# JiehongLin/SAM-6D

Hardware: AMD Instinct MI355X
Metric: RGB-D frames/sec (SAM-6D per-frame hot path: SAM ViT-H encoder + ISM scoring + PEM) (higher is better)
Workload: dtype bf16 (SAM ViT-H: 87 % of the step) + f16 (PEM ViT-B feature extractor) + f32 (ISM scoring, PEM point transformer and pose solvers); 1 GPU; LM-O single object: 32 frames/step/GPU, 640x480 RGB-D -> 1024^2 SAM input, P=128 proposals x 42 templates (scored in groups of 8 frames), 1 instance/frame, 2048 pts (PEM batch 32); sam_frames_per_launch_group=16, pem_vit_dtype=fp16 (set by bench.py; the library default is fp32)

## Files before the change

### sam6d_amd/csrc/s6d_attn_common.h

```cpp
#pragma once
#include "s6d_bf16.h"

#ifndef S6D_ATTN_F16
#define S6D_ATTN_F16 0
#endif
#if S6D_ATTN_F16
#define S6D_ATTN_NS s6d_h
#define S6D_ATTN_MFMA16(a, b, c) __builtin_amdgcn_mfma_f32_16x16x32_f16(a, b, c, 0, 0, 0)
#define S6D_ATTN_ONE 0x3C00
#else
#define S6D_ATTN_NS s6d
#define S6D_ATTN_MFMA16(a, b, c) __builtin_amdgcn_mfma_f32_16x16x32_bf16(a, b, c, 0, 0, 0)
#define S6D_ATTN_ONE 0x3F80
#endif

namespace S6D_ATTN_NS {
using namespace s6d;

#if S6D_ATTN_F16
typedef f16x8 bf16x8;
__device__ __forceinline__ u16 f2bf(float f) {
  union { _Float16 b; u16 u; } x;
  x.b = (_Float16)f;
  return x.u;
}
__device__ __forceinline__ float bf2f(u16 h) {
  union { _Float16 b; u16 u; } x;
  x.u = h;
  return (float)x.b;
}
#else
__device__ __forceinline__ u16 f2bf(float f) { return bf16_bits(f); }
__device__ __forceinline__ float bf2f(u16 h) { return bf16_value(h); }
#endif

struct AttnParams {
  const u16 *qkv;
  const u16 *qkv_bias;
  const u16 *rel_h;
  const u16 *rel_w;
  u16 *out;
  int B, H, W, nh;
  int ws;
  int S;
  int T;
  int nwx, nwy;
  int LT;
  unsigned magicS;
  float scale_log2;
  long tok_stride, which_stride, head_stride;
};

__device__ __forceinline__ const u16 *qkv_at(const AttnParams &p, size_t tok, int which, int head) {
  return p.qkv + tok * (size_t)p.tok_stride + (size_t)which * (size_t)p.which_stride + (size_t)head * (size_t)p.head_stride;
}

#ifndef S6D_ATTN_ABLATE
#define S6D_ATTN_ABLATE 0
#endif
constexpr int kAbl = S6D_ATTN_ABLATE;
#ifndef S6D_G64_TIMING
#define S6D_G64_TIMING 0
#endif
#if S6D_G64_TIMING
#define S6D_TICK(tk, i)                                  \
  do {                                                   \
    __builtin_amdgcn_sched_barrier(0);                   \
    (tk)[i] = (long long)__builtin_amdgcn_s_memtime();   \
    __builtin_amdgcn_sched_barrier(0);                   \
  } while (0)
#else
#define S6D_TICK(tk, i) do { } while (0)
#endif

constexpr float kLog2e = 1.4426950408889634f;
__device__ __forceinline__ float fast_exp2(float x) { return __builtin_amdgcn_exp2f(x); }

template <int HD>
struct Cfg {
  static constexpr int KS = (HD + 31) / 32;
  static constexpr int HDP = KS * 32;
  static constexpr int DT = HD / 16;
  static constexpr int KROW = HDP + 8;
  static constexpr int VROW = HD == 64 ? HD + 8 : (((HD + 15) / 16) | 1) * 16;
  static constexpr int KT = 64;
  static constexpr int KPARTS = HDP / 8, VPARTS = HD / 8;
};

__device__ __forceinline__ int div_S(const AttnParams &p, int n) { return (int)__umulhi((unsigned)n, p.magicS); }

__device__ __forceinline__ bool token_offset(const AttnParams &p, int b, int wy, int wx, int t, size_t &off) {
  if (p.ws == 0) {
    off = (size_t)b * p.T + min(t, p.T - 1);
    return t < p.T;
  }
  const int ty = div_S(p, t), tx = t - ty * p.S;
  const int y = wy * p.ws + ty, x = wx * p.ws + tx;
  const bool in = (y < p.H) && (x < p.W) && (t < p.T);
  off = (in || p.qkv_bias) ? ((size_t)(b * p.H + min(y, p.H - 1)) * p.W + min(x, p.W - 1)) : (size_t)b * p.H * p.W;
  return in;
}

template <int HD>
__device__ __forceinline__ uint4 load_chunk(const AttnParams &p, int which, int head, bool valid, size_t tok, int d0) {
  const int C = p.nh * HD;
  const int dc = d0 < HD ? d0 : HD - 8;
  const u16 *a = qkv_at(p, tok, which, head) + dc;
  const u16 *bsrc = p.qkv_bias ? p.qkv_bias + (size_t)which * C + head * HD + dc : a;
  const uint4 v = *reinterpret_cast<const uint4 *>(valid ? a : bsrc);
  return d0 < HD ? v : make_uint4(0, 0, 0, 0);
}

template <int HD, int NS>
struct StripState {
  bf16x8 qf[NS][Cfg<HD>::KS];
  float twr[NS][16];
  float m_run[NS];
  f32x4 lacc[NS];
  f32x4 oacc[NS][Cfg<HD>::DT];
  const float *th[NS], *tw[NS];
  int qy[NS], qx[NS];
};

template <int HD, int MODE, int NS, bool KSWZ = false, bool PRIO = false, int SUBS = 4>
__device__ __forceinline__ void process_tile(const AttnParams &p, const u16 *Kl, const u16 *Vl, int key0,
                                             StripState<HD, NS> &st, const float (&thv)[NS], int lane, long long *tk = nullptr) {
  using C = Cfg<HD>;
  static_assert(SUBS >= 1 && SUBS <= 4, "a tile has four 16-key sub-tiles");
  const int g = lane >> 4, c = lane & 15;
  const int gk = KSWZ ? (g ^ kswz(c)) : g;
  float s[NS][4][4];
  if (PRIO) __builtin_amdgcn_s_setprio(1);
  auto kfrag = [&](int sub, int ks) __attribute__((always_inline)) {
    return *reinterpret_cast<const bf16x8 *>(Kl + (sub * 16 + c) * C::KROW + ks * 32 + gk * 8);
  };
#pragma unroll
  for (int sub = 0; sub < 4; ++sub) {
    f32x4 acc[NS];
#pragma unroll
    for (int n = 0; n < NS; ++n) acc[n] = f32x4{0.f, 0.f, 0.f, 0.f};
    if (sub >= SUBS) {
#pragma unroll
      for (int n = 0; n < NS; ++n)
#pragma unroll
        for (int r = 0; r < 4; ++r) s[n][sub][r] = -1e30f;
      continue;
    }
    if (!(kAbl & 16)) {
#pragma unroll
      for (int ks = 0; ks < C::KS; ++ks) {
        const bf16x8 a = kfrag(sub, ks);
#pragma unroll
        for (int n = 0; n < NS; ++n) acc[n] = S6D_ATTN_MFMA16(a, st.qf[n][ks], acc[n]);
      }
    }
#pragma unroll
    for (int n = 0; n < NS; ++n)
#pragma unroll
      for (int r = 0; r < 4; ++r) {
        float v = acc[n][r] * p.scale_log2;
        if (MODE == 1) {
          s[n][sub][r] = v + st.twr[n][sub * 4 + r];
        } else {
          const int kk = key0 + sub * 16 + g * 4 + r;
          if (MODE == 0) {
            const int ky = div_S(p, kk), kx = kk - ky * p.S;
            const int jh = min(max(st.qy[n] - ky + p.S - 1, 0), p.LT - 1), jw = st.qx[n] - kx + p.S - 1;
            v += st.th[n][c * p.LT + jh] + st.tw[n][c * p.LT + jw];
          }
          s[n][sub][r] = kk < p.T ? v : -1e30f;
        }
      }
  }
  union PB { bf16x8 v; u16 h[8]; };
  PB pb[NS][2];
  union VA { bf16x8 v; s16x4 q[2]; };
  if (PRIO) __builtin_amdgcn_s_setprio(0);
  if (kAbl & 4) {
#pragma unroll
    for (int n = 0; n < NS; ++n)
#pragma unroll
      for (int sub = 0; sub < 4; ++sub)
#pragma unroll
        for (int r = 0; r < 4; ++r) pb[n][sub >> 1].h[(sub & 1) * 4 + r] = f2bf(s[n][sub][r]);
  } else {
    constexpr float kDefer = 6.0f;
    float mx[NS];
    bool grow[NS], any_grow = false;
#pragma unroll
    for (int n = 0; n < NS; ++n) {
      float v = s[n][0][0];
#pragma unroll
      for (int sub = 0; sub < SUBS; ++sub)
#pragma unroll
        for (int r = 0; r < 4; ++r) v = fmaxf(v, s[n][sub][r]);
      v = fmaxf(v, __shfl_xor(v, 16));
      v = fmaxf(v, __shfl_xor(v, 32));
      if (MODE == 1) v += thv[n];
      mx[n] = v;
      grow[n] = __any(v - st.m_run[n] > kDefer);
      any_grow |= grow[n];
    }
    S6D_TICK(tk, 3);
    if (any_grow) {
#pragma unroll
      for (int n = 0; n < NS; ++n)
        if (grow[n]) {
          const float m_new = fmaxf(st.m_run[n], mx[n]);
          const float alpha = fast_exp2(st.m_run[n] - m_new);
          st.lacc[n] *= alpha;
#pragma unroll
          for (int dt = 0; dt < C::DT; ++dt) st.oacc[n][dt] *= alpha;
          st.m_run[n] = m_new;
        }
    }
#pragma unroll
    for (int n = 0; n < NS; ++n) {
      const float m_sub = (MODE == 1) ? st.m_run[n] - thv[n] : st.m_run[n];
#pragma unroll
      for (int sub = 0; sub < 4; ++sub)
#pragma unroll
        for (int r = 0; r < 4; ++r)
          pb[n][sub >> 1].h[(sub & 1) * 4 + r] = sub < SUBS ? f2bf(fast_exp2(s[n][sub][r] - m_sub)) : (u16)0;
    }
  }
  if (kAbl & 8) {
#pragma unroll
    for (int n = 0; n < NS; ++n) st.lacc[n][0] += (float)pb[n][0].h[0] + (float)pb[n][1].h[7];
    return;
  }
  union { bf16x8 v; u16 h[8]; } ones;
#pragma unroll
  for (int i = 0; i < 8; ++i) ones.h[i] = S6D_ATTN_ONE;
  S6D_TICK(tk, 4);
  if (PRIO) __builtin_amdgcn_s_setprio(1);
#pragma unroll
  for (int j = 0; j < (SUBS + 1) / 2; ++j) {
    const u16 *vrow = Vl + (32 * j + g * 4 + (c >> 2)) * C::VROW + (c & 3) * 4;
#pragma unroll
    for (int n = 0; n < NS; ++n) st.lacc[n] = S6D_ATTN_MFMA16(ones.v, pb[n][j].v, st.lacc[n]);
#pragma unroll
    for (int dt = 0; dt < C::DT; ++dt) {
      VA va;
      va.q[0] = __builtin_amdgcn_ds_read_tr16_b64_v4i16((S6D_LDS(s16x4) *)(vrow + dt * 16));
      va.q[1] = __builtin_amdgcn_ds_read_tr16_b64_v4i16((S6D_LDS(s16x4) *)(vrow + 16 * C::VROW + dt * 16));
#pragma unroll
      for (int n = 0; n < NS; ++n)
        st.oacc[n][dt] = S6D_ATTN_MFMA16(va.v, pb[n][j].v, st.oacc[n][dt]);
    }
  }
  if (PRIO) __builtin_amdgcn_s_setprio(0);
}

constexpr float kNoMaxSumLimit = 1.2676506e30f;
constexpr float kNoMaxFinite = 3.0e38f;

template <int HD, int NS, bool KSWZ>
__device__ __forceinline__ void process_tile_nomax(const AttnParams &p, const u16 *Kl, const u16 *Vl, StripState<HD, NS> &st,
                                                   const f32x4 (&cbias)[NS][4], const float (&nb)[NS], int lane) {
  using C = Cfg<HD>;
  const int g = lane >> 4, c = lane & 15;
  const int gk = KSWZ ? (g ^ kswz(c)) : g;
  union PB { bf16x8 v; u16 h[8]; };
  PB pb[NS][2];
#pragma unroll
  for (int sub = 0; sub < 4; ++sub) {
    f32x4 acc[NS];
#pragma unroll
    for (int n = 0; n < NS; ++n) acc[n] = cbias[n][sub];
#pragma unroll
    for (int ks = 0; ks < C::KS; ++ks) {
      const bf16x8 a = *reinterpret_cast<const bf16x8 *>(Kl + (sub * 16 + c) * C::KROW + ks * 32 + gk * 8);
#pragma unroll
      for (int n = 0; n < NS; ++n) acc[n] = S6D_ATTN_MFMA16(a, st.qf[n][ks], acc[n]);
    }
#pragma unroll
    for (int n = 0; n < NS; ++n)
#pragma unroll
      for (int r = 0; r < 4; ++r)
        pb[n][sub >> 1].h[(sub & 1) * 4 + r] = f2bf(fast_exp2(__builtin_fmaf(acc[n][r], p.scale_log2, nb[n])));
  }
  union { bf16x8 v; u16 h[8]; } ones;
#pragma unroll
  for (int i = 0; i < 8; ++i) ones.h[i] = S6D_ATTN_ONE;
  union VA { bf16x8 v; s16x4 q[2]; };
#pragma unroll
  for (int j = 0; j < 2; ++j) {
    const u16 *vrow = Vl + (32 * j + g * 4 + (c >> 2)) * C::VROW + (c & 3) * 4;
#pragma unroll
    for (int n = 0; n < NS; ++n) st.lacc[n] = S6D_ATTN_MFMA16(ones.v, pb[n][j].v, st.lacc[n]);
#pragma unroll
    for (int dt = 0; dt < C::DT; ++dt) {
      VA va;
      va.q[0] = __builtin_amdgcn_ds_read_tr16_b64_v4i16((S6D_LDS(s16x4) *)(vrow + dt * 16));
      va.q[1] = __builtin_amdgcn_ds_read_tr16_b64_v4i16((S6D_LDS(s16x4) *)(vrow + 16 * C::VROW + dt * 16));
#pragma unroll
      for (int n = 0; n < NS; ++n) st.oacc[n][dt] = S6D_ATTN_MFMA16(va.v, pb[n][j].v, st.oacc[n][dt]);
    }
  }
}

template <int HD, int THREADS>
struct Stager {
  using C = Cfg<HD>;
  static constexpr int NK = (64 * C::KPARTS + THREADS - 1) / THREADS;
  static constexpr int NV = (64 * C::VPARTS + THREADS - 1) / THREADS;
  uint4 k[NK], v[NV];

  __device__ __forceinline__ void load(const AttnParams &p, int b, int wy, int wx, int head, int key0, int tid) {
#pragma unroll
    for (int n = 0; n < NK; ++n) {
      const int i = min(tid + n * THREADS, 64 * C::KPARTS - 1);
      const int key = i / C::KPARTS, part = i - key * C::KPARTS;
      size_t tok;
      const bool valid = token_offset(p, b, wy, wx, key0 + key, tok);
      k[n] = load_chunk<HD>(p, 1, head, valid, tok, part * 8);
    }
#pragma unroll
    for (int n = 0; n < NV; ++n) {
      const int i = min(tid + n * THREADS, 64 * C::VPARTS - 1);
      const int key = i / C::VPARTS, part = i - key * C::VPARTS;
      size_t tok;
      const bool valid = token_offset(p, b, wy, wx, key0 + key, tok);
      v[n] = load_chunk<HD>(p, 2, head, valid, tok, part * 8);
    }
  }
  __device__ __forceinline__ void store(u16 *Kl, u16 *Vl, int tid, int klim = 64, int vlim = 64) const {
#pragma unroll
    for (int n = 0; n < NK; ++n) {
      const int i = tid + n * THREADS;
      const int key = i / C::KPARTS, part = i - key * C::KPARTS;
      if (i < 64 * C::KPARTS && key < klim) *reinterpret_cast<uint4 *>(Kl + key * C::KROW + part * 8) = k[n];
    }
#pragma unroll
    for (int n = 0; n < NV; ++n) {
      const int i = tid + n * THREADS;
      const int key = i / C::VPARTS, part = i - key * C::VPARTS;
      if (i < 64 * C::VPARTS && key < vlim) *reinterpret_cast<uint4 *>(Vl + key * C::VROW + part * 8) = v[n];
    }
  }
};

template <int HD, int THREADS>
struct StagerLinear {
  using C = Cfg<HD>;
  static constexpr int NK = (64 * C::KPARTS + THREADS - 1) / THREADS;
  static constexpr int NV = (64 * C::VPARTS + THREADS - 1) / THREADS;
  uint4 k[NK], v[NV];
  const u16 *kp[NK], *vp[NV];
  int ko[NK], vo[NV];
  bool kz[NK];
  static_assert(Cfg<HD>::KROW - Cfg<HD>::HDP == 8, "K rows end in a 16-byte pad");

  __device__ __forceinline__ void init(const AttnParams &p, int b, int head, int tid) {
#pragma unroll
    for (int n = 0; n < NK; ++n) {
      const int i = tid + n * THREADS, ic = min(i, 64 * C::KPARTS - 1);
      const int key = ic / C::KPARTS, part = ic - key * C::KPARTS;
      kz[n] = part * 8 >= HD;
      kp[n] = qkv_at(p, (size_t)b * p.T + key, 1, head) + (kz[n] ? HD - 8 : part * 8);
      ko[n] = i < 64 * C::KPARTS ? key * C::KROW + (part ^ kswz(key)) * 8 : (tid & 63) * C::KROW + C::HDP;
    }
#pragma unroll
    for (int n = 0; n < NV; ++n) {
      const int i = tid + n * THREADS, ic = min(i, 64 * C::VPARTS - 1);
      const int key = ic / C::VPARTS, part = ic - key * C::VPARTS;
      vp[n] = qkv_at(p, (size_t)b * p.T + key, 2, head) + part * 8;
      vo[n] = i < 64 * C::VPARTS ? 64 * C::KROW + key * C::VROW + part * 8 : (tid & 63) * C::KROW + C::HDP;
    }
  }
  __device__ __forceinline__ void load(size_t tile_stride_elems, int t) {
#pragma unroll
    for (int n = 0; n < NK; ++n) k[n] = *reinterpret_cast<const uint4 *>(kp[n] + tile_stride_elems * t);
#pragma unroll
    for (int n = 0; n < NV; ++n) v[n] = *reinterpret_cast<const uint4 *>(vp[n] + tile_stride_elems * t);
  }
  __device__ __forceinline__ void store(u16 *Kl) const {
#pragma unroll
    for (int n = 0; n < NK; ++n) *reinterpret_cast<uint4 *>(Kl + ko[n]) = kz[n] ? make_uint4(0, 0, 0, 0) : k[n];
#pragma unroll
    for (int n = 0; n < NV; ++n) *reinterpret_cast<uint4 *>(Kl + vo[n]) = v[n];
  }
};

template <int HD>
__device__ __forceinline__ void load_q(const AttnParams &p, int b, int wy, int wx, int head, int q0,
                                       bf16x8 (&qf)[Cfg<HD>::KS], int lane) {
  const int g = lane >> 4, c = lane & 15;
  size_t tok;
  const bool valid = token_offset(p, b, wy, wx, q0 + c, tok);
#pragma unroll
  for (int ks = 0; ks < Cfg<HD>::KS; ++ks) {
    union { uint4 u; bf16x8 v; } x;
    x.u = load_chunk<HD>(p, 0, head, valid, tok, ks * 32 + g * 8);
    qf[ks] = x.v;
  }
}

template <int HD, int NJT>
__device__ __forceinline__ void build_table(const u16 *rel, int j0, int sgn, const bf16x8 (&qf)[Cfg<HD>::KS],
                                            float *dst, int ld, int lane) {
  using C = Cfg<HD>;
  const int g = lane >> 4, c = lane & 15;
  union { uint4 u; bf16x8 v; } r[NJT][C::KS];
#pragma unroll
  for (int jt = 0; jt < NJT; ++jt) {
    const int j = j0 + sgn * (jt * 16 + c);
#pragma unroll
    for (int ks = 0; ks < C::KS; ++ks)
      r[jt][ks].u = *reinterpret_cast<const uint4 *>(rel + (size_t)j * C::HDP + ks * 32 + g * 8);
  }
#pragma unroll
  for (int jt = 0; jt < NJT; ++jt) {
    f32x4 a = {0.f, 0.f, 0.f, 0.f};
#pragma unroll
    for (int ks = 0; ks < C::KS; ++ks) a = S6D_ATTN_MFMA16(r[jt][ks].v, qf[ks], a);
    float *o = dst + c * ld + jt * 16 + g * 4;
    if ((ld & 3) == 0) {
      *reinterpret_cast<float4 *>(o) = make_float4(a[0] * kLog2e, a[1] * kLog2e, a[2] * kLog2e, a[3] * kLog2e);
    } else {
#pragma unroll
      for (int r = 0; r < 4; ++r) o[r] = a[r] * kLog2e;
    }
  }
}

template <int HD>
__device__ __forceinline__ void store_strip(const AttnParams &p, int b, int wy, int wx, int head, int q0, float l_run,
                                            const f32x4 (&oacc)[Cfg<HD>::DT], int lane) {
  const int g = lane >> 4, c = lane & 15;
  size_t tok;
  if (!token_offset(p, b, wy, wx, q0 + c, tok)) return;
  const float inv = 1.0f / l_run;
  u16 *dst = p.out + tok * (size_t)(p.nh * HD) + head * HD;
#pragma unroll
  for (int dt = 0; dt < Cfg<HD>::DT; ++dt) {
    union { uint2 u; u16 h[4]; } o;
#pragma unroll
    for (int r = 0; r < 4; ++r) o.h[r] = f2bf(oacc[dt][r] * inv);
    *reinterpret_cast<uint2 *>(dst + dt * 16 + g * 4) = o.u;
  }
}

struct WinItem {
  int b, wy, wx, head;
  __device__ __forceinline__ void decode(const AttnParams &p, int id) {
    const int nwin = p.B * p.nwy * p.nwx, cut = (nwin & ~7) * p.nh;
    int win;
    if (id < cut) {
      const int xcd = id & 7, loc = id >> 3;
      head = loc % p.nh;
      win = (loc / p.nh) * 8 + xcd;
    } else {
      head = id % p.nh;
      win = id / p.nh;
    }
    wx = win % p.nwx; win /= p.nwx;
    wy = win % p.nwy; win /= p.nwy;
    b = win;
  }
};

__device__ const uint4 g_attn_zero16 = {0u, 0u, 0u, 0u};

template <class... P, class... A>
static void launch_lds(void (*kernel)(P...), unsigned grid, unsigned block, size_t lds, hipStream_t st, A... args) {
  (void)hipFuncSetAttribute(reinterpret_cast<const void *>(kernel), hipFuncAttributeMaxDynamicSharedMemorySize, (int)lds);
  hipLaunchKernelGGL(kernel, dim3(grid), dim3(block), lds, st, args...);
}

}
```

### sam6d_amd/csrc/s6d_attn_global.h

```cpp
#pragma once
#include "s6d_attn_common.h"

namespace S6D_ATTN_NS {

constexpr bool kGlbPrio = true;

template <int HD, int WAVES, int MODE>
__global__ __launch_bounds__(WAVES * 64) void attn_global_kernel(AttnParams p) {
  using C = Cfg<HD>;
  constexpr int NS = 2;
  static_assert(MODE == 0 || MODE == 2, "attn_global_kernel: table bias (0) or no bias (2); the 64 x 64 grid is attn_global64_kernel's");
  S6D_DYN_LDS(smem);
  constexpr int KBYTES = 64 * C::KROW * 2, VBYTES = 64 * C::VROW * 2;
  auto Kbuf = [&](int r) { return reinterpret_cast<u16 *>(smem + r * (KBYTES + VBYTES)); };
  auto Vbuf = [&](int r) { return reinterpret_cast<u16 *>(smem + r * (KBYTES + VBYTES) + KBYTES); };
  float *tabs = reinterpret_cast<float *>(smem + 2 * (KBYTES + VBYTES));
  const int tid = threadIdx.x, wave = tid >> 6, lane = tid & 63;
  const int c = lane & 15;

  const int nqt = (p.T + WAVES * 16 * NS - 1) / (WAVES * 16 * NS);
  int id = blockIdx.x;
  const int nbh = p.B * p.nh;
  int qt, bh;
  if ((nbh & 7) == 0) {
    const int xcd = id & 7, loc = id >> 3;
    qt = loc % nqt;
    bh = (loc / nqt) * 8 + xcd;
  } else {
    qt = id % nqt;
    bh = id / nqt;
  }
  const int head = bh % p.nh, b = bh / p.nh;
  StripState<HD, NS> st;
  int q0[NS];
#pragma unroll
  for (int n = 0; n < NS; ++n) {
    q0[n] = ((qt * WAVES + wave) * NS + n) * 16;
    load_q<HD>(p, b, 0, 0, head, q0[n], st.qf[n], lane);
    const int qi = min(q0[n] + c, p.T - 1);
    st.qy[n] = div_S(p, qi);
    st.qx[n] = qi - st.qy[n] * p.S;
    st.m_run[n] = -1e30f;
    st.lacc[n] = f32x4{0.f, 0.f, 0.f, 0.f};
#pragma unroll
    for (int i = 0; i < 16; ++i) st.twr[n][i] = 0.f;
#pragma unroll
    for (int dt = 0; dt < C::DT; ++dt) st.oacc[n][dt] = f32x4{0.f, 0.f, 0.f, 0.f};
    st.th[n] = nullptr;
    st.tw[n] = nullptr;
  }
  if (MODE == 0) {
#pragma unroll
    for (int n = 0; n < NS; ++n) {
      float *th = tabs + (size_t)(wave * NS + n) * 2 * 16 * p.LT, *tw = th + 16 * p.LT;
      for (int jt = 0; jt < p.LT / 16; ++jt) {
        build_table<HD, 1>(p.rel_h, jt * 16, 1, st.qf[n], th + jt * 16, p.LT, lane);
        build_table<HD, 1>(p.rel_w, jt * 16, 1, st.qf[n], tw + jt * 16, p.LT, lane);
      }
      st.th[n] = th;
      st.tw[n] = tw;
    }
  }
  const int ntile = p.T / 64;
  StagerLinear<HD, WAVES * 64> sg;
  sg.init(p, b, head, tid);
  const size_t tstride = (size_t)64 * (size_t)p.tok_stride;
  sg.load(tstride, 0);
  __syncthreads();
  sg.store(Kbuf(0));
  __syncthreads();
  auto tile = [&](int t) {
    const float thv[NS] = {0.f, 0.f};
    if (!(kAbl & 2)) process_tile<HD, MODE, NS, true, kGlbPrio>(p, Kbuf(t & 1), Vbuf(t & 1), t * 64, st, thv, lane);
  };
  for (int t = 0; t + 1 < ntile; ++t) {
    if (!(kAbl & 1)) sg.load(tstride, t + 1);
    tile(t);
    if (!(kAbl & 32)) sg.store(Kbuf((t & 1) ^ 1));
    __syncthreads();
  }
  tile(ntile - 1);
#pragma unroll
  for (int n = 0; n < NS; ++n) store_strip<HD>(p, b, 0, 0, head, q0[n], st.lacc[n][0], st.oacc[n], lane);
}

constexpr int G64_THLD = 65;
#ifndef S6D_G64_SLOTS
#define S6D_G64_SLOTS 3
#endif
#ifndef S6D_G64_WAVES
#define S6D_G64_WAVES 8
#endif
#ifndef S6D_G64_NOMAX
#define S6D_G64_NOMAX 1
#endif

template <int HD, int WAVES_, int SLOTS_>
struct G64 {
  using C = Cfg<HD>;
  static constexpr int WAVES = WAVES_, NS = 2, SLOTS = SLOTS_;
  static constexpr int KCH = C::KROW / 8, VCH = C::VROW / 8;
  static constexpr int NPIECE = KCH + VCH;
  static constexpr int PW = (NPIECE + WAVES - 1) / WAVES;
  static constexpr int SLOT = NPIECE * 1024;
  static constexpr int RING = SLOTS * SLOT;
  static constexpr int TABS = WAVES * NS * 16 * G64_THLD * 4;
  static constexpr int LDS = RING + TABS + 16;
  static_assert(NPIECE > WAVES * (PW - 1) && PW >= 2, "every wave has a real piece to repeat");
  static_assert(RING >= WAVES * 16 * 80 * 4, "the prologue's per-wave scratch aliases the ring");
  static_assert(PW * (SLOTS - 2) <= 15 || SLOTS == 2, "vmcnt immediates used below");
};

template <int PW>
__device__ __forceinline__ void g64_wait_tiles(int n) {
  switch (PW * n) {
#define S6D_G64_CASE(k) case k: S6D_VMCNT(k); break;
    S6D_G64_CASE(0) S6D_G64_CASE(3) S6D_G64_CASE(5) S6D_G64_CASE(6) S6D_G64_CASE(9) S6D_G64_CASE(10) S6D_G64_CASE(12)
#undef S6D_G64_CASE
    default: S6D_VMCNT(15); break;
  }
}

template <int HD, int WAVES, int SLOTS>
__global__ __launch_bounds__(WAVES * 64) void attn_global64_kernel(AttnParams p) {
  using C = Cfg<HD>;
  using G = G64<HD, WAVES, SLOTS>;
  constexpr int NS = G::NS, PW = G::PW;
  S6D_DYN_LDS(smem);
  float *tabs = reinterpret_cast<float *>(smem + G::RING);
  const int tid = threadIdx.x, wave = __builtin_amdgcn_readfirstlane(tid >> 6), lane = tid & 63;
  const int g = lane >> 4, c = lane & 15;
  const int nqt = p.T / (WAVES * 16 * NS);
  const int nbh = p.B * p.nh;
  int id = blockIdx.x, qt, bh;
  if ((nbh & 7) == 0) {
    const int xcd = id & 7, loc = id >> 3;
    qt = loc % nqt;
    bh = (loc / nqt) * 8 + xcd;
  } else {
    qt = id % nqt;
    bh = id / nqt;
  }
  const int head = bh % p.nh, b = bh / p.nh;
  StripState<HD, NS> st;
  int q0[NS];
  float *thm[NS];
#pragma unroll
  for (int n = 0; n < NS; ++n) {
    q0[n] = ((qt * WAVES + wave) * NS + n) * 16;
    load_q<HD>(p, b, 0, 0, head, q0[n], st.qf[n], lane);
    st.qy[n] = q0[n] >> 6;
    st.qx[n] = (q0[n] & 63) + c;
    st.m_run[n] = -1e30f;
    st.lacc[n] = f32x4{0.f, 0.f, 0.f, 0.f};
#pragma unroll
    for (int dt = 0; dt < C::DT; ++dt) st.oacc[n][dt] = f32x4{0.f, 0.f, 0.f, 0.f};
    st.th[n] = nullptr;
    st.tw[n] = nullptr;
    float *th = tabs + (size_t)(wave * NS + n) * 16 * G64_THLD;
    float *Gs = reinterpret_cast<float *>(smem) + (size_t)wave * 16 * 80;
    const int q0y = q0[n] >> 6, q0x = q0[n] & 63;
    build_table<HD, 4>(p.rel_h, q0y + 63, -1, st.qf[n], th, G64_THLD, lane);
    build_table<HD, 5>(p.rel_w, q0x, 1, st.qf[n], Gs, 80, lane);
    S6D_WAVE_RENDEZVOUS();
#pragma unroll
    for (int sub = 0; sub < 4; ++sub)
#pragma unroll
      for (int r = 0; r < 4; ++r) st.twr[n][sub * 4 + r] = Gs[c * 80 + (c + 63 - (sub * 16 + g * 4 + r))];
    S6D_WAVE_RENDEZVOUS();
    thm[n] = th;
  }
  const u16 *src[PW];
  long inc[PW];
  int dsto[PW];
  const long tstride = 64L * p.tok_stride;
#pragma unroll
  for (int i = 0; i < PW; ++i) {
    const int q = wave + WAVES * i < G::NPIECE ? wave + WAVES * i : wave + WAVES * (i - 1);
    const bool isk = q < G::KCH;
    const int piece = isk ? q : q - G::KCH, rowch = isk ? G::KCH : G::VCH;
    const int j = piece * 64 + lane;
    const int row = j / rowch, pp = j - row * rowch;
    const int part = isk ? (pp < C::KPARTS ? pp ^ kswz(row) : C::KPARTS) : pp;
    const bool data = part * 8 < HD;
    src[i] = data ? qkv_at(p, (size_t)b * p.T + row, isk ? 1 : 2, head) + part * 8 : reinterpret_cast<const u16 *>(&g_attn_zero16);
    inc[i] = data ? tstride : 0;
    dsto[i] = q * 1024;
  }
  auto issue = [&](int slot) __attribute__((always_inline)) {
#pragma unroll
    for (int i = 0; i < PW; ++i) {
      S6D_LDS(char) *dst = (S6D_LDS(char) *)smem + slot * G::SLOT + dsto[i];
      lds_dma16_m0(src[i], dst);
      src[i] += inc[i];
    }
  };
  const int ntile = p.T / 64;
  constexpr int D = SLOTS - 1;
  static_assert(D >= 1 && D <= 6, "ring depth");
  f32x4 cbias[NS][4];
  {
    const float inv = 1.0f / p.scale_log2;
#pragma unroll
    for (int n = 0; n < NS; ++n)
#pragma unroll
      for (int sub = 0; sub < 4; ++sub)
#pragma unroll
        for (int r = 0; r < 4; ++r) cbias[n][sub][r] = st.twr[n][sub * 4 + r] * inv;
  }
  int *redo = reinterpret_cast<int *>(smem + G::RING + G::TABS);
  const u16 *src0[PW];
#pragma unroll
  for (int i = 0; i < PW; ++i) src0[i] = src[i];
  long long tk[6] = {0, 0, 0, 0, 0, 0}, tsum[5] = {0, 0, 0, 0, 0};
  int slot = 0;
  auto tile_head = [&](int t, float (&thv)[NS]) __attribute__((always_inline)) -> const u16 * {
    S6D_TICK(tk, 0);
    g64_wait_tiles<PW>(min(D - 1, ntile - 1 - t));
    S6D_LGKM0();
    __builtin_amdgcn_s_barrier();
    S6D_TICK(tk, 1);
    if (t + D < ntile && !(kAbl & 1)) issue(slot >= 1 ? slot - 1 : SLOTS - 1);
#pragma unroll
    for (int n = 0; n < NS; ++n) thv[n] = thm[n][c * G64_THLD + t];
    S6D_TICK(tk, 2);
    const u16 *Kl = reinterpret_cast<const u16 *>(smem + slot * G::SLOT);
    slot = slot == SLOTS - 1 ? 0 : slot + 1;
    return Kl;
  };
  auto prime = [&]() __attribute__((always_inline)) {
    __syncthreads();
    if (tid == 0) *redo = 0;
#pragma unroll
    for (int d = 0; d < D; ++d) issue(d);
    slot = 0;
  };
  bool done = false;
  if (S6D_G64_NOMAX && !S6D_G64_TIMING) {
    prime();
    {
      float thv[NS];
      const u16 *Kl = tile_head(0, thv);
      process_tile<HD, 1, NS, true, kGlbPrio>(p, Kl, Kl + 64 * C::KROW, 0, st, thv, lane, tk);
    }
    for (int t = 1; t < ntile; ++t) {
      float thv[NS], nb[NS];
      const u16 *Kl = tile_head(t, thv);
#pragma unroll
      for (int n = 0; n < NS; ++n) nb[n] = thv[n] - st.m_run[n];
      process_tile_nomax<HD, NS, true>(p, Kl, Kl + 64 * C::KROW, st, cbias, nb, lane);
    }
    bool bad = false;
#pragma unroll
    for (int n = 0; n < NS; ++n) {
      bad |= !(st.lacc[n][0] < kNoMaxSumLimit);
#pragma unroll
      for (int dt = 0; dt < C::DT; ++dt)
#pragma unroll
        for (int r = 0; r < 4; ++r) bad |= !(fabsf(st.oacc[n][dt][r]) < kNoMaxFinite);
    }
    if (__any(bad) && lane == 0) *redo = 1;
    __syncthreads();
    done = *redo == 0;
    if (!done) {
#pragma unroll
      for (int n = 0; n < NS; ++n) {
        st.m_run[n] = -1e30f;
        st.lacc[n] = f32x4{0.f, 0.f, 0.f, 0.f};
#pragma unroll
        for (int dt = 0; dt < C::DT; ++dt) st.oacc[n][dt] = f32x4{0.f, 0.f, 0.f, 0.f};
      }
#pragma unroll
      for (int i = 0; i < PW; ++i) src[i] = src0[i];
    }
  }
  if (!done) {
    prime();
    for (int t = 0; t < ntile; ++t) {
      float thv[NS];
      const u16 *Kl = tile_head(t, thv);
      if (!(kAbl & 2)) process_tile<HD, 1, NS, true, kGlbPrio>(p, Kl, Kl + 64 * C::KROW, t * 64, st, thv, lane, tk);
      S6D_TICK(tk, 5);
      if (S6D_G64_TIMING)
#pragma unroll
        for (int i = 0; i < 5; ++i) tsum[i] += tk[i + 1] - tk[i];
    }
  }
#pragma unroll
  for (int n = 0; n < NS; ++n) store_strip<HD>(p, b, 0, 0, head, q0[n], st.lacc[n][0], st.oacc[n], lane);
  if (S6D_G64_TIMING && blockIdx.x == 8 && lane == 0) {
    long long *dbg = reinterpret_cast<long long *>(p.out + (size_t)p.B * p.T * p.nh * HD);
#pragma unroll
    for (int i = 0; i < 5; ++i) dbg[wave * 5 + i] = tsum[i];
  }
}

template <int HD>
static int launch_global(AttnParams p, hipStream_t st) {
  using C = Cfg<HD>;
  const bool bias = p.rel_h != nullptr;
  if (p.T % 64 != 0) return S6D_EUNSUPPORTED;
  if (bias && p.S == 64) {
    using G = G64<HD, S6D_G64_WAVES, S6D_G64_SLOTS>;
    static_assert(G::LDS <= 160 * 1024, "ring + tables fit the CU's LDS");
    launch_lds(attn_global64_kernel<HD, G::WAVES, G::SLOTS>, (unsigned)(p.B * p.nh * (p.T / (G::WAVES * 32))), G::WAVES * 64, G::LDS, st, p);
    return launch_status();
  }
  constexpr int WAVES = 4, NS = 2;
  const size_t ring = (size_t)2 * 64 * (C::KROW + C::VROW) * 2;
  const int nqt = (p.T + WAVES * 16 * NS - 1) / (WAVES * 16 * NS);
  const unsigned grid = (unsigned)(p.B * p.nh * nqt);
  const size_t lds = bias ? ring + (size_t)WAVES * NS * 2 * 16 * p.LT * 4 : ring;
  if (lds > 160 * 1024) return S6D_EUNSUPPORTED;
  if (bias) {
    launch_lds(attn_global_kernel<HD, WAVES, 0>, grid, WAVES * 64, lds, st, p);
  } else {
    launch_lds(attn_global_kernel<HD, WAVES, 2>, grid, WAVES * 64, lds, st, p);
  }
  return launch_status();
}

}
```

Measured before the change: 164.0 frames/s.

## Use 32x32 MFMA tiles in the 64x64 global attention kernel

Adds a 32x32x16 bf16 MFMA path for the global-attention kernel with relative-position bias when the head dim is 16 mod 32 (ViT-H, HD=80). Each wave now processes one 32-query tile instead of two 16-row strips, with new K/V LDS row layouts. V is padded with ones so the row sum falls out of the PV matmul as an extra column. This aims to cut instruction count and LDS traffic per FLOP, at the cost of more accumulator registers (possible occupancy loss) and extra padded columns of wasted MFMA work.

```diff
diff --git a/sam6d_amd/csrc/s6d_attn_common.h b/sam6d_amd/csrc/s6d_attn_common.h
--- a/sam6d_amd/csrc/s6d_attn_common.h
+++ b/sam6d_amd/csrc/s6d_attn_common.h
@@ -13,6 +13,15 @@
 #define S6D_ATTN_MFMA16(a, b, c) __builtin_amdgcn_mfma_f32_16x16x32_bf16(a, b, c, 0, 0, 0)
 #define S6D_ATTN_ONE 0x3F80
 #endif
+
+#ifndef S6D_ATTN_MI
+#define S6D_ATTN_MI 32
+#endif
+#ifndef S6D_G64_MI
+#define S6D_G64_MI S6D_ATTN_MI
+#endif
+static_assert((S6D_ATTN_MI == 16 || S6D_ATTN_MI == 32) && (S6D_G64_MI == 16 || S6D_G64_MI == 32), "matrix instruction shape: 16 or 32");
+#define S6D_ATTN_MFMA32(a, b, c) __builtin_amdgcn_mfma_f32_32x32x16_bf16(a, b, c, 0, 0, 0)
 
 namespace S6D_ATTN_NS {
 using namespace s6d;
diff --git a/sam6d_amd/csrc/s6d_attn_global.h b/sam6d_amd/csrc/s6d_attn_global.h
--- a/sam6d_amd/csrc/s6d_attn_global.h
+++ b/sam6d_amd/csrc/s6d_attn_global.h
@@ -84,6 +84,127 @@
   for (int n = 0; n < NS; ++n) store_strip<HD>(p, b, 0, 0, head, q0[n], st.lacc[n][0], st.oacc[n], lane);
 }
 
+#if S6D_G64_MI == 32
+__device__ const uint4 g_attn_one16 = {0x3F803F80u, 0x3F803F80u, 0x3F803F80u, 0x3F803F80u};
+#endif
+__device__ __forceinline__ constexpr int mi32_row(int i, int h) { return (i & 3) + 8 * (i >> 2) + 4 * h; }
+union PB32 { bf16x8 v; u16 h[8]; };
+
+template <int HD>
+struct Tile32State {
+  static constexpr int KS = HD / 16, DT = HD / 32 + 1;
+  bf16x8 qf[KS];
+  f32x16 cb[2];
+  float m_run;
+  f32x16 oacc[DT];
+  __device__ __forceinline__ void reset() {
+    m_run = -1e30f;
+#pragma unroll
+    for (int dt = 0; dt < DT; ++dt)
+#pragma unroll
+      for (int i = 0; i < 16; ++i) oacc[dt][i] = 0.f;
+  }
+  __device__ __forceinline__ float row_sum() const { return oacc[DT - 1][8]; }
+  __device__ __forceinline__ bool out_of_range() const {
+    bool bad = !(row_sum() < kNoMaxSumLimit);
+#pragma unroll
+    for (int dt = 0; dt < DT; ++dt)
+#pragma unroll
+      for (int i = 0; i < 16; ++i) bad |= !(fabsf(oacc[dt][i]) < kNoMaxFinite);
+    return bad;
+  }
+};
+
+template <int HD, int KROW>
+__device__ __forceinline__ f32x16 qk_tile32(const u16 *Kl, int kt, const Tile32State<HD> &st, int lane) {
+  const u16 *krow = Kl + (kt * 32 + (lane & 31)) * KROW + (lane >> 5) * 8;
+  f32x16 acc = st.cb[kt];
+#pragma unroll
+  for (int ks = 0; ks < Tile32State<HD>::KS; ++ks)
+    acc = S6D_ATTN_MFMA32(*reinterpret_cast<const bf16x8 *>(krow + ks * 16), st.qf[ks], acc);
+  return acc;
+}
+
+template <int HD, int VROW>
+__device__ __forceinline__ void pv_tile32(const u16 *Vl, const PB32 (&pb)[2][2], Tile32State<HD> &st, int lane) {
+  const int c = lane & 15;
+  const u16 *vrow = Vl + ((lane >> 5) * 4 + (c >> 2)) * VROW + ((lane >> 4) & 1) * 16 + (c & 3) * 4;
+  union VA { bf16x8 v; s16x4 q[2]; };
+#pragma unroll
+  for (int j = 0; j < 4; ++j)
+#pragma unroll
+    for (int dt = 0; dt < Tile32State<HD>::DT; ++dt) {
+      VA va;
+      va.q[0] = __builtin_amdgcn_ds_read_tr16_b64_v4i16((S6D_LDS(s16x4) *)(vrow + (16 * j) * VROW + dt * 32));
+      va.q[1] = __builtin_amdgcn_ds_read_tr16_b64_v4i16((S6D_LDS(s16x4) *)(vrow + (16 * j + 8) * VROW + dt * 32));
+      st.oacc[dt] = S6D_ATTN_MFMA32(va.v, pb[j >> 1][j & 1].v, st.oacc[dt]);
+    }
+}
+
+template <int HD, int KROW, int VROW, bool PRIO>
+__device__ __forceinline__ void process_tile32(const AttnParams &p, const u16 *Kl, const u16 *Vl, Tile32State<HD> &st, float thv,
+                                               int lane, long long *tk = nullptr) {
+  f32x16 s[2];
+  if (PRIO) __builtin_amdgcn_s_setprio(1);
+#pragma unroll
+  for (int kt = 0; kt < 2; ++kt) s[kt] = qk_tile32<HD, KROW>(Kl, kt, st, lane) * p.scale_log2;
+  if (PRIO) __builtin_amdgcn_s_setprio(0);
+  constexpr float kDefer = 6.0f;
+  float v = s[0][0];
+#pragma unroll
+  for (int kt = 0; kt < 2; ++kt)
+#pragma unroll
+    for (int i = 0; i < 16; ++i) v = fmaxf(v, s[kt][i]);
+  v = fmaxf(v, __shfl_xor(v, 32)) + thv;
+  S6D_TICK(tk, 3);
+  if (__any(v - st.m_run > kDefer)) {
+    const float m_new = fmaxf(st.m_run, v);
+    const float alpha = fast_exp2(st.m_run - m_new);
+#pragma unroll
+    for (int dt = 0; dt < Tile32State<HD>::DT; ++dt) st.oacc[dt] *= alpha;
+    st.m_run = m_new;
+  }
+  const float m_sub = st.m_run - thv;
+  PB32 pb[2][2];
+#pragma unroll
+  for (int kt = 0; kt < 2; ++kt)
+#pragma unroll
+    for (int i = 0; i < 16; ++i) pb[kt][i >> 3].h[i & 7] = f2bf(fast_exp2(s[kt][i] - m_sub));
+  S6D_TICK(tk, 4);
+  if (PRIO) __builtin_amdgcn_s_setprio(1);
+  pv_tile32<HD, VROW>(Vl, pb, st, lane);
+  if (PRIO) __builtin_amdgcn_s_setprio(0);
+}
+
+template <int HD, int KROW, int VROW>
+__device__ __forceinline__ void process_tile32_nomax(const AttnParams &p, const u16 *Kl, const u16 *Vl, Tile32State<HD> &st, float nb,
+                                                     int lane) {
+  PB32 pb[2][2];
+#pragma unroll
+  for (int kt = 0; kt < 2; ++kt) {
+    const f32x16 acc = qk_tile32<HD, KROW>(Kl, kt, st, lane);
+#pragma unroll
+    for (int i = 0; i < 16; ++i) pb[kt][i >> 3].h[i & 7] = f2bf(fast_exp2(__builtin_fmaf(acc[i], p.scale_log2, nb)));
+  }
+  pv_tile32<HD, VROW>(Vl, pb, st, lane);
+}
+
+template <int HD>
+__device__ __forceinline__ void store_tile32(const AttnParams &p, int b, int head, int q0, const Tile32State<HD> &st, int lane) {
+  const float inv = 1.0f / st.row_sum();
+  u16 *dst = p.out + ((size_t)b * p.T + q0 + (lane & 31)) * (size_t)(p.nh * HD) + head * HD + (lane >> 5) * 4;
+#pragma unroll
+  for (int dt = 0; dt < Tile32State<HD>::DT; ++dt)
+#pragma unroll
+    for (int m = 0; m < 4; ++m) {
+      if (dt * 32 + m * 8 >= HD) continue;
+      union { uint2 u; u16 h[4]; } o;
+#pragma unroll
+      for (int r = 0; r < 4; ++r) o.h[r] = f2bf(st.oacc[dt][m * 4 + r] * inv);
+      *reinterpret_cast<uint2 *>(dst + dt * 32 + m * 8) = o.u;
+    }
+}
+
 constexpr int G64_THLD = 65;
 #ifndef S6D_G64_SLOTS
 #define S6D_G64_SLOTS 3
@@ -99,7 +220,9 @@
 struct G64 {
   using C = Cfg<HD>;
   static constexpr int WAVES = WAVES_, NS = 2, SLOTS = SLOTS_;
-  static constexpr int KCH = C::KROW / 8, VCH = C::VROW / 8;
+  static constexpr bool MI32 = S6D_G64_MI == 32 && HD % 32 == 16;
+  static constexpr int KROW = MI32 ? HD + 8 : C::KROW, VROW = MI32 ? HD + 16 : C::VROW;
+  static constexpr int KCH = KROW / 8, VCH = VROW / 8;
   static constexpr int NPIECE = KCH + VCH;
   static constexpr int PW = (NPIECE + WAVES - 1) / WAVES;
   static constexpr int SLOT = NPIECE * 1024;
@@ -142,33 +265,68 @@
     bh = id / nqt;
   }
   const int head = bh % p.nh, b = bh / p.nh;
+  constexpr bool MI32 = G::MI32;
+  constexpr int NT = MI32 ? 1 : NS;
   StripState<HD, NS> st;
+  Tile32State<HD> s32;
   int q0[NS];
-  float *thm[NS];
-#pragma unroll
-  for (int n = 0; n < NS; ++n) {
-    q0[n] = ((qt * WAVES + wave) * NS + n) * 16;
-    load_q<HD>(p, b, 0, 0, head, q0[n], st.qf[n], lane);
-    st.qy[n] = q0[n] >> 6;
-    st.qx[n] = (q0[n] & 63) + c;
-    st.m_run[n] = -1e30f;
-    st.lacc[n] = f32x4{0.f, 0.f, 0.f, 0.f};
-#pragma unroll
-    for (int dt = 0; dt < C::DT; ++dt) st.oacc[n][dt] = f32x4{0.f, 0.f, 0.f, 0.f};
-    st.th[n] = nullptr;
-    st.tw[n] = nullptr;
-    float *th = tabs + (size_t)(wave * NS + n) * 16 * G64_THLD;
+  float *thm[NT];
+  if constexpr (!MI32) {
+#pragma unroll
+    for (int n = 0; n < NS; ++n) {
+      q0[n] = ((qt * WAVES + wave) * NS + n) * 16;
+      load_q<HD>(p, b, 0, 0, head, q0[n], st.qf[n], lane);
+      st.qy[n] = q0[n] >> 6;
+      st.qx[n] = (q0[n] & 63) + c;
+      st.m_run[n] = -1e30f;
+      st.lacc[n] = f32x4{0.f, 0.f, 0.f, 0.f};
+#pragma unroll
+      for (int dt = 0; dt < C::DT; ++dt) st.oacc[n][dt] = f32x4{0.f, 0.f, 0.f, 0.f};
+      st.th[n] = nullptr;
+      st.tw[n] = nullptr;
+      float *th = tabs + (size_t)(wave * NS + n) * 16 * G64_THLD;
+      float *Gs = reinterpret_cast<float *>(smem) + (size_t)wave * 16 * 80;
+      const int q0y = q0[n] >> 6, q0x = q0[n] & 63;
+      build_table<HD, 4>(p.rel_h, q0y + 63, -1, st.qf[n], th, G64_THLD, lane);
+      build_table<HD, 5>(p.rel_w, q0x, 1, st.qf[n], Gs, 80, lane);
+      S6D_WAVE_RENDEZVOUS();
+#pragma unroll
+      for (int sub = 0; sub < 4; ++sub)
+#pragma unroll
+        for (int r = 0; r < 4; ++r) st.twr[n][sub * 4 + r] = Gs[c * 80 + (c + 63 - (sub * 16 + g * 4 + r))];
+      S6D_WAVE_RENDEZVOUS();
+      thm[n] = th;
+    }
+  } else {
+    const int q0w = (qt * WAVES + wave) * 32, r = lane & 31, h = lane >> 5;
+    const float inv = 1.0f / p.scale_log2;
     float *Gs = reinterpret_cast<float *>(smem) + (size_t)wave * 16 * 80;
-    const int q0y = q0[n] >> 6, q0x = q0[n] & 63;
-    build_table<HD, 4>(p.rel_h, q0y + 63, -1, st.qf[n], th, G64_THLD, lane);
-    build_table<HD, 5>(p.rel_w, q0x, 1, st.qf[n], Gs, 80, lane);
-    S6D_WAVE_RENDEZVOUS();
-#pragma unroll
-    for (int sub = 0; sub < 4; ++sub)
-#pragma unroll
-      for (int r = 0; r < 4; ++r) st.twr[n][sub * 4 + r] = Gs[c * 80 + (c + 63 - (sub * 16 + g * 4 + r))];
-    S6D_WAVE_RENDEZVOUS();
-    thm[n] = th;
+    q0[0] = q0w;
+#pragma unroll
+    for (int n = 0; n < NS; ++n) {
+      bf16x8 qf16[C::KS];
+      const int q0n = q0w + n * 16;
+      load_q<HD>(p, b, 0, 0, head, q0n, qf16, lane);
+      build_table<HD, 4>(p.rel_h, (q0n >> 6) + 63, -1, qf16, tabs + (size_t)(wave * NS + n) * 16 * G64_THLD, G64_THLD, lane);
+      build_table<HD, 5>(p.rel_w, q0n & 63, 1, qf16, Gs, 80, lane);
+      S6D_WAVE_RENDEZVOUS();
+#pragma unroll
+      for (int kt = 0; kt < 2; ++kt)
+#pragma unroll
+        for (int i = 0; i < 16; ++i) {
+          const float v = Gs[c * 80 + (c + 63 - (kt * 32 + mi32_row(i, h)))] * inv;
+          s32.cb[kt][i] = n == 0 || (r >> 4) == n ? v : s32.cb[kt][i];
+        }
+      S6D_WAVE_RENDEZVOUS();
+    }
+    thm[0] = tabs + (size_t)wave * 32 * G64_THLD;
+#pragma unroll
+    for (int ks = 0; ks < Tile32State<HD>::KS; ++ks) {
+      union { uint4 u; bf16x8 v; } x;
+      x.u = load_chunk<HD>(p, 0, head, true, (size_t)b * p.T + q0w + r, ks * 16 + h * 8);
+      s32.qf[ks] = x.v;
+    }
+    s32.reset();
   }
   const u16 *src[PW];
   long inc[PW];
@@ -181,9 +339,13 @@
     const int piece = isk ? q : q - G::KCH, rowch = isk ? G::KCH : G::VCH;
     const int j = piece * 64 + lane;
     const int row = j / rowch, pp = j - row * rowch;
-    const int part = isk ? (pp < C::KPARTS ? pp ^ kswz(row) : C::KPARTS) : pp;
+    const int part = isk ? (MI32 ? pp : pp < C::KPARTS ? pp ^ kswz(row) : C::KPARTS) : pp;
     const bool data = part * 8 < HD;
-    src[i] = data ? qkv_at(p, (size_t)b * p.T + row, isk ? 1 : 2, head) + part * 8 : reinterpret_cast<const u16 *>(&g_attn_zero16);
+    const u16 *fill = reinterpret_cast<const u16 *>(&g_attn_zero16);
+#if S6D_G64_MI == 32
+    if (MI32 && !isk) fill = reinterpret_cast<const u16 *>(&g_attn_one16);
+#endif
+    src[i] = data ? qkv_at(p, (size_t)b * p.T + row, isk ? 1 : 2, head) + part * 8 : fill;
     inc[i] = data ? tstride : 0;
     dsto[i] = q * 1024;
   }
@@ -199,7 +361,7 @@
   constexpr int D = SLOTS - 1;
   static_assert(D >= 1 && D <= 6, "ring depth");
   f32x4 cbias[NS][4];
-  {
+  if constexpr (!MI32) {
     const float inv = 1.0f / p.scale_log2;
 #pragma unroll
     for (int n = 0; n < NS; ++n)
@@ -214,7 +376,8 @@
   for (int i = 0; i < PW; ++i) src0[i] = src[i];
   long long tk[6] = {0, 0, 0, 0, 0, 0}, tsum[5] = {0, 0, 0, 0, 0};
   int slot = 0;
-  auto tile_head = [&](int t, float (&thv)[NS]) __attribute__((always_inline)) -> const u16 * {
+  const int trow = MI32 ? lane & 31 : c;
+  auto tile_head = [&](int t, float (&thv)[NT]) __attribute__((always_inline)) -> const u16 * {
     S6D_TICK(tk, 0);
     g64_wait_tiles<PW>(min(D - 1, ntile - 1 - t));
     S6D_LGKM0();
@@ -222,7 +385,7 @@
     S6D_TICK(tk, 1);
     if (t + D < ntile && !(kAbl & 1)) issue(slot >= 1 ? slot - 1 : SLOTS - 1);
 #pragma unroll
-    for (int n = 0; n < NS; ++n) thv[n] = thm[n][c * G64_THLD + t];
+    for (int n = 0; n < NT; ++n) thv[n] = thm[n][trow * G64_THLD + t];
     S6D_TICK(tk, 2);
     const u16 *Kl = reinterpret_cast<const u16 *>(smem + slot * G::SLOT);
     slot = slot == SLOTS - 1 ? 0 : slot + 1;
@@ -238,37 +401,55 @@
   bool done = false;
   if (S6D_G64_NOMAX && !S6D_G64_TIMING) {
     prime();
-    {
-      float thv[NS];
+    if constexpr (MI32) {
+      float thv[NT];
       const u16 *Kl = tile_head(0, thv);
-      process_tile<HD, 1, NS, true, kGlbPrio>(p, Kl, Kl + 64 * C::KROW, 0, st, thv, lane, tk);
-    }
-    for (int t = 1; t < ntile; ++t) {
-      float thv[NS], nb[NS];
-      const u16 *Kl = tile_head(t, thv);
-#pragma unroll
-      for (int n = 0; n < NS; ++n) nb[n] = thv[n] - st.m_run[n];
-      process_tile_nomax<HD, NS, true>(p, Kl, Kl + 64 * C::KROW, st, cbias, nb, lane);
+      process_tile32<HD, G::KROW, G::VROW, kGlbPrio>(p, Kl, Kl + 64 * G::KROW, s32, thv[0], lane, tk);
+      for (int t = 1; t < ntile; ++t) {
+        Kl = tile_head(t, thv);
+        process_tile32_nomax<HD, G::KROW, G::VROW>(p, Kl, Kl + 64 * G::KROW, s32, thv[0] - s32.m_run, lane);
+      }
+    } else {
+      {
+        float thv[NS];
+        const u16 *Kl = tile_head(0, thv);
+        process_tile<HD, 1, NS, true, kGlbPrio>(p, Kl, Kl + 64 * C::KROW, 0, st, thv, lane, tk);
+      }
+      for (int t = 1; t < ntile; ++t) {
+        float thv[NS], nb[NS];
+        const u16 *Kl = tile_head(t, thv);
+#pragma unroll
+        for (int n = 0; n < NS; ++n) nb[n] = thv[n] - st.m_run[n];
+        process_tile_nomax<HD, NS, true>(p, Kl, Kl + 64 * C::KROW, st, cbias, nb, lane);
+      }
     }
     bool bad = false;
-#pragma unroll
-    for (int n = 0; n < NS; ++n) {
-      bad |= !(st.lacc[n][0] < kNoMaxSumLimit);
-#pragma unroll
-      for (int dt = 0; dt < C::DT; ++dt)
-#pragma unroll
-        for (int r = 0; r < 4; ++r) bad |= !(fabsf(st.oacc[n][dt][r]) < kNoMaxFinite);
+    if constexpr (MI32) {
+      bad = s32.out_of_range();
+    } else {
+#pragma unroll
+      for (int n = 0; n < NS; ++n) {
+        bad |= !(st.lacc[n][0] < kNoMaxSumLimit);
+#pragma unroll
+        for (int dt = 0; dt < C::DT; ++dt)
+#pragma unroll
+          for (int r = 0; r < 4; ++r) bad |= !(fabsf(st.oacc[n][dt][r]) < kNoMaxFinite);
+      }
     }
     if (__any(bad) && lane == 0) *redo = 1;
     __syncthreads();
     done = *redo == 0;
     if (!done) {
-#pragma unroll
-      for (int n = 0; n < NS; ++n) {
-        st.m_run[n] = -1e30f;
-        st.lacc[n] = f32x4{0.f, 0.f, 0.f, 0.f};
-#pragma unroll
-        for (int dt = 0; dt < C::DT; ++dt) st.oacc[n][dt] = f32x4{0.f, 0.f, 0.f, 0.f};
+      if constexpr (MI32) {
+        s32.reset();
+      } else {
+#pragma unroll
+        for (int n = 0; n < NS; ++n) {
+          st.m_run[n] = -1e30f;
+          st.lacc[n] = f32x4{0.f, 0.f, 0.f, 0.f};
+#pragma unroll
+          for (int dt = 0; dt < C::DT; ++dt) st.oacc[n][dt] = f32x4{0.f, 0.f, 0.f, 0.f};
+        }
       }
 #pragma unroll
       for (int i = 0; i < PW; ++i) src[i] = src0[i];
@@ -277,17 +458,27 @@
   if (!done) {
     prime();
     for (int t = 0; t < ntile; ++t) {
-      float thv[NS];
+      float thv[NT];
       const u16 *Kl = tile_head(t, thv);
-      if (!(kAbl & 2)) process_tile<HD, 1, NS, true, kGlbPrio>(p, Kl, Kl + 64 * C::KROW, t * 64, st, thv, lane, tk);
+      if (!(kAbl & 2)) {
+        if constexpr (MI32) {
+          process_tile32<HD, G::KROW, G::VROW, kGlbPrio>(p, Kl, Kl + 64 * G::KROW, s32, thv[0], lane, tk);
+        } else {
+          process_tile<HD, 1, NS, true, kGlbPrio>(p, Kl, Kl + 64 * C::KROW, t * 64, st, thv, lane, tk);
+        }
+      }
       S6D_TICK(tk, 5);
       if (S6D_G64_TIMING)
 #pragma unroll
         for (int i = 0; i < 5; ++i) tsum[i] += tk[i + 1] - tk[i];
     }
   }
-#pragma unroll
-  for (int n = 0; n < NS; ++n) store_strip<HD>(p, b, 0, 0, head, q0[n], st.lacc[n][0], st.oacc[n], lane);
+  if constexpr (MI32) {
+    store_tile32<HD>(p, b, head, q0[0], s32, lane);
+  } else {
+#pragma unroll
+    for (int n = 0; n < NS; ++n) store_strip<HD>(p, b, 0, 0, head, q0[n], st.lacc[n][0], st.oacc[n], lane);
+  }
   if (S6D_G64_TIMING && blockIdx.x == 8 && lane == 0) {
     long long *dbg = reinterpret_cast<long long *>(p.out + (size_t)p.B * p.T * p.nh * HD);
 #pragma unroll
```

Measured after the change: 165.5 frames/s (median of 6 runs). Within noise of the previous version (+0.9%).
